# yynps737/zero-latency-yolo

Measured on AMD Instinct MI355X. Metric: frames_per_sec, higher is better.
Workload: dtype bf16; 1 GPU; YOLOv8-nano 416x416 batch=64 throughput path (BASELINE configs[2]), bf16; engines_per_gpu=3, weights=seeded synthetic (no real weights offline), graph=True, parallelism=single GPU

## Files before the change

### zero-latency-yolo_amd/csrc/engine.cpp

```cpp
#include "zly_internal.h"
#include "weights.h"

#include <algorithm>
#include <atomic>
#include <chrono>
#include <condition_variable>
#include <deque>
#include <map>
#include <mutex>
#include <string>
#include <thread>
#include <type_traits>
#include <vector>
#include <string.h>
#include <stdio.h>
#include <stdlib.h>

namespace zly {

static thread_local std::string g_last_error;

static int fail(int code, const std::string& msg) { g_last_error = msg; return code; }

#define HIP_TRY(expr, code)                                                                        \
// ... 2392 lines not shown
    HIP_TRY(hipMemcpyAsync(out, e->d_scratch_f32, elems * sizeof(float), hipMemcpyDeviceToHost, e->stream), ZLY_ERR_INFERENCE);
    HIP_TRY(hipStreamSynchronize(e->stream), ZLY_ERR_INFERENCE);
    if (c) *c = C;
    if (h) *h = b.H;
    if (w) *w = b.W;
    return ZLY_OK;
}

int32_t zly_num_classes(const zly_engine* e) { return e ? e->nc : 0; }
int32_t zly_weights_fp8(const zly_engine* e) { return (e && e->model.fp8_weights) ? 1 : 0; }
int32_t zly_num_anchors(const zly_engine* e) { return e ? e->N : 0; }
int32_t zly_num_ops(const zly_engine* e) { return e ? (int32_t)e->ops.size() : 0; }

int32_t zly_op_info_at(const zly_engine* e, int32_t i, zly_op_info* out)
{
    if (!e || !out || i < 0 || i >= (int32_t)e->ops.size()) return fail(ZLY_ERR_INVALID_ARGUMENT, "bad argument");
    const Op& op = e->ops[(size_t)i];
    memset(out, 0, sizeof *out);
    snprintf(out->name, sizeof out->name, "%s", op.name.c_str());
    out->kind = op.kind;
    out->flops_per_frame = op.flops;
    out->bytes_per_frame = op.bytes;
    return ZLY_OK;
}

int32_t zly_op_kernel_name(zly_engine* e, int32_t i, int32_t n, char* out, size_t cap)
{
    if (!e || !out || cap < 8 || i < 0 || i >= (int32_t)e->ops.size() || n < 1 || n > e->cfg.max_batch) return fail(ZLY_ERR_INVALID_ARGUMENT, "bad argument");
    std::lock_guard<std::mutex> lk(e->mu);
    const std::vector<Launch>& t = resolve_launches(e, n);
    const Launch& L = t[(size_t)i];
    const Op& op = e->ops[(size_t)i];
    std::string k;
    switch (L.kind) {
    case LK_NONE:
        switch (t[(size_t)L.covered_by].kind) {
        case LK_STEM: case LK_STEM1: k = op.kind == OP_PREPROCESS ? "(fused into stem_fused_kernel)" : "(fused into the previous launch)"; break;
        case LK_PAIR: case LK_WS_PAIR: k = "(fused into the previous launch)"; break;
        case LK_C2F: k = "(fused into the C2f kernel at " + e->ops[(size_t)L.covered_by].name + ")"; break;
        case LK_SPPF_FUSED: k = "(fused into the SPPF kernel at model.9.cv1)"; break;
        case LK_MULTI: k = "(in a merged Detect launch)"; break;
        case LK_HEAD: k = op.kind == OP_CONV ? "(computed in the Detect tail at surviving anchors)" : "(covered by the last tail launch)"; break;
        }
        break;
    case LK_PREPROCESS: k = L.lb ? "preprocess_kernel<LB> (letterbox)" : "preprocess_kernel"; break;
    case LK_STEM: k = L.lb ? "stem_fused_kernel<LB> (letterbox)" : "stem_fused_kernel"; break;
    case LK_STEM1: k = L.lb ? "stem_model1_kernel<LB> (letterbox preprocess+model.0+model.1)" : "stem_model1_kernel (preprocess+model.0+model.1)"; break;
    case LK_SPPF_POOL: k = L.pool16 ? "sppf_pool16_kernel<DPP row windows, one barrier>" : "sppf_pool_kernel"; break;
    case LK_SPPF_FUSED: k = "sppf_fused_kernel<cv1+3 pools+cv2,SPLIT=" + std::to_string(sppf_split(e->ops[(size_t)e->sppf_cv2].cout, n, e->sw)) + ">"; break;
    case LK_MULTI: k = L.multi_ct == 3 ? "conv_igemm_multi_kernel<CT=3> (the 3 Detect stems)" : "conv_igemm_multi_kernel<CT=2> (the 6 Detect branch convs)"; break;
    case LK_C2F: {
        const C2fGroup& g = e->c2fs[(size_t)op.c2f];
        k = "c2f_kernel<C=" + std::to_string(g.c) + (g.c == 32 ? ",NW=" + std::to_string(L.c2f.nw) : std::string()) +
            (g.mode == 3 ? ",cv1+bottleneck+cv2>" : g.mode == 1 ? ",cv1+bottleneck>" : ",bottleneck+cv2>");
        break;
    }
    case LK_PAIR: k = "bottleneck_pair_kernel<" + std::to_string(e->pairs[(size_t)op.pair].c) + ">"; break;
    case LK_WS_PAIR: k = std::string("conv3x3_ws_pair_kernel<") + (e->pairs[(size_t)op.pair].res ? "RES," : "") + "64->64->64," + std::to_string(L.ws_pair.g.TH) + "x" + std::to_string(L.ws_pair.g.TW) + " tiles>"; break;
    case LK_CONV_WSK: k = "conv3x3_wsk_kernel<K=720 packed across taps,5 channel tiles>"; break;
    case LK_CONV: {
        const int cin = op.in.C + (op.in2.buf >= 0 ? op.in2.C : 0);
        const ConvPlan& c = L.conv;
        switch (c.kind) {
        case CONV_WS1: k = std::string("conv1x1_ws_kernel<") + (op.in2.buf >= 0 ? "dual-source," : "") + "NK=" + std::to_string(cin / 32) + "," + std::to_string(c.ct) + " channel tiles," + std::to_string(c.pt * 16) + " px>"; break;
        case CONV_WS: k = std::string("conv3x3_ws_kernel<") + (op.stride == 2 ? "S=2," : "") + (c.rowt ? "ROWT," : "") + (c.tpw1 ? "TPW=1," : "TPW=2,") + std::to_string(c.ct) + " channel tiles>"; break;
        case CONV_LDS: k = "conv3x3_lds_kernel<S=" + std::to_string(op.stride) + ",CT=" + std::to_string(c.ct) + ",PT=" + std::to_string(c.pt) + (c.wres ? ",wres>" : ">"); break;
        case CONV_STREAM: k = "conv1x1_stream_kernel<CT=" + std::to_string(c.ct) + ",PT=" + std::to_string(c.pt) + ",NK=" + std::to_string((cin + 31) / 32) + ">"; break;
        default: k = std::string("conv_igemm_kernel<") + (op.ks == 1 ? (op.in2.buf >= 0 ? "1x1 dual-source" : "1x1") : (c.fastk ? "3x3" : "3x3 generic-K")) +
                 ",CT=" + std::to_string(c.ct) + ",PT=" + std::to_string(c.pt) + ",KSPLIT=" + std::to_string(c.ksplit) + ">";
        }
        break;
    }
    case LK_HEAD: {
        k = L.lb ? "head_fused_kernel<LB> (letterbox box mapping)" : "head_fused_kernel";
        std::string lv;
        for (int l = 0; l < 3; ++l)
            if (L.box_mode[l] && (L.only_level < 0 || L.only_level == l)) lv += std::string(lv.empty() ? "" : ",") + "P" + std::to_string(3 + l) + (L.box_mode[l] == 1 ? ":ws" : ":lds");
        if (!lv.empty()) k += " (+ box conv in k-step order " + lv + ")";
        break;
    }
    case LK_NMS: k = "nms_kernel"; break;
    }
    snprintf(out, cap, "%s", k.c_str());
    return ZLY_OK;
}

int32_t zly_launch_info_at(zly_engine* e, int32_t i, int32_t n, zly_launch_info* out)
{
    if (!e || !out || i < 0 || i >= (int32_t)e->ops.size() || n < 1 || n > e->cfg.max_batch) return fail(ZLY_ERR_INVALID_ARGUMENT, "bad argument");
    std::lock_guard<std::mutex> lk(e->mu);
    memset(out, 0, sizeof *out);
    const int nops = (int)e->ops.size();
    const std::vector<Launch>& t = resolve_launches(e, n);
    out->covered_by = t[(size_t)i].covered_by;
    if (out->covered_by != i) return ZLY_OK;
    std::vector<char> in_group((size_t)nops, 0);
    for (int j = 0; j < nops; ++j) in_group[(size_t)j] = t[(size_t)j].covered_by == i ? 1 : 0;
    std::map<int, std::vector<char>> written_in, read_out, counted_in, counted_out;
    auto chan = [&](std::map<int, std::vector<char>>& m, int buf) -> std::vector<char>& {
        std::vector<char>& v = m[buf];
        if (v.empty()) v.assign((size_t)e->bufs[(size_t)buf].C + 64, 0);
        return v;
    };
    std::vector<IoView> io;
    for (int j = 0; j < nops; ++j) {
        io.clear();
        if (in_group[(size_t)j]) { op_writes(e, e->ops[(size_t)j], &io); for (const IoView& v : io) for (int c = 0; c < v.C; ++c) chan(written_in, v.buf)[(size_t)(v.co + c)] = 1; }
// ... 108 lines not shown
```

### zero-latency-yolo_amd/csrc/kernels_pair.hip

```cpp
#include "zly_internal.h"
#include "conv_device.h"
#include <stdlib.h>
#include <stdio.h>

namespace zly {

typedef __attribute__((ext_vector_type(4))) short s16x4;
typedef __attribute__((ext_vector_type(4))) unsigned int u32x4_t;

template <int C> struct PairGeom;
template <> struct PairGeom<16> {
    static constexpr int CT = 1, KS = 1, FRAGB = 8, PITCH = 48, WTILE = 512;
    static constexpr bool WRES = true;
    typedef s16x4 frag;
    static __device__ __forceinline__ f32x4 mma(frag a, frag b, f32x4 c) { return __builtin_amdgcn_mfma_f32_16x16x16bf16_1k(a, b, c, 0, 0, 0); }
};
template <> struct PairGeom<32> {
    static constexpr int CT = 2, KS = 1, FRAGB = 16, PITCH = 96, WTILE = 1024;
    static constexpr bool WRES = true;
    typedef bf16x8 frag;
    static __device__ __forceinline__ f32x4 mma(frag a, frag b, f32x4 c) { return __builtin_amdgcn_mfma_f32_16x16x32_bf16(a, b, c, 0, 0, 0); }
};
template <> struct PairGeom<64> {
    static constexpr int CT = 4, KS = 2, FRAGB = 16, PITCH = 160, WTILE = 1024;
    static constexpr bool WRES = false;
    typedef bf16x8 frag;
    static __device__ __forceinline__ f32x4 mma(frag a, frag b, f32x4 c) { return __builtin_amdgcn_mfma_f32_16x16x32_bf16(a, b, c, 0, 0, 0); }
};

__device__ __forceinline__ int div_small(int q, float inv) { return (int)(((float)q + 0.5f) * inv); }

template <int C>
__device__ __forceinline__ void pair_taps(const unsigned char* __restrict__ src, const unsigned char* __restrict__ lw, int off, int rowb, int lane,
                                          f32x4 (&acc)[PairGeom<C>::CT])
{
    typedef PairGeom<C> G;
    typedef typename G::frag F;
#pragma unroll
    for (int c = 0; c < G::CT; ++c) acc[c] = f32x4{0.f, 0.f, 0.f, 0.f};
    const unsigned char* wl = lw + lane * G::FRAGB;
    const int kxo[3] = {0, G::FRAGB == 8 ? opaque_offset(G::PITCH) : G::PITCH, G::FRAGB == 8 ? opaque_offset(2 * G::PITCH) : 2 * G::PITCH};
#pragma unroll
    for (int ky = 0; ky < 3; ++ky) {
        const unsigned char* row = src + off + ky * rowb;
#pragma unroll
        for (int kx = 0; kx < 3; ++kx) {
#pragma unroll
            for (int ks = 0; ks < G::KS; ++ks) {
                const F x = *reinterpret_cast<const F*>(row + (G::FRAGB == 8 ? kxo[kx] : kx * G::PITCH) + ks * 64);
#pragma unroll
                for (int c = 0; c < G::CT; ++c) {
                    const F w = *reinterpret_cast<const F*>(wl + ((c * 9 + ky * 3 + kx) * G::KS + ks) * G::WTILE);
                    acc[c] = G::mma(w, x, acc[c]);
                }
            }
        }
// ... 121 lines not shown
            stage_weights(lwB, a.wB);
            __syncthreads();
        }

        for (int t = wave; t < ntB; t += NW) {
            if (C == 64) asm volatile("" ::: "memory");
            const int q = t * 16 + p;
            const int qc = min(q, NPB - 1);
            const int oy = div_small(qc, invTW), ox = qc - oy * a.TW;
            f32x4 acc[G::CT];
            pair_taps<C>(lmid, lwB, (oy * MW + ox) * G::PITCH + kq * G::FRAGB, MW * G::PITCH, lane, acc);
            f32x4 o[G::CT];
#pragma unroll
            for (int c = 0; c < G::CT; ++c) {
                f32x4 v = acc[c] + biasB[c];
#pragma unroll
                for (int r = 0; r < 4; ++r) v[r] = silu<bf16_t>(v[r]);
                o[c] = v;
            }
            const int gy = y0 + oy, gx = x0 + ox;
            if (q < NPB && gy < a.H && gx < a.W) {
                const unsigned char* xs = lin + ((oy + 2) * PW + ox + 2) * G::PITCH;
                bf16_t* dst = out + ((size_t)(b * a.H + gy) * a.W + gx) * a.out_cs;
                if (C == 16) {
                    if (a.res) o[0] += load4(reinterpret_cast<const bf16_t*>(xs) + kq * 4);
                    store4(dst + kq * 4, o[0]);
                } else {
#pragma unroll
                    for (int g2 = 0; g2 < G::CT / 2; ++g2) {
                        f32x4 lo = o[2 * g2], hi = o[(2 * g2 + 1) % G::CT];
                        if (a.res) {
                            f32x4 ra, rb;
                            load8(reinterpret_cast<const bf16_t*>(xs) + g2 * 32 + kq * 8, ra, rb);
                            lo += ra; hi += rb;
                        }
                        store8(dst + g2 * 32 + kq * 8, lo, hi);
                    }
                }
            }
        }
        if (tnext >= a.total_tiles) break;
        tl = tnext;
        __syncthreads();
    }
}

#ifdef ZLY_C2F_DIAG
__device__ unsigned long long* g_c2f_diag = nullptr;
#define C2FSTAMP(k) do { __builtin_amdgcn_sched_barrier(0); unsigned long long t_; asm volatile("s_memtime %0\n\ts_waitcnt lgkmcnt(0)" : "=s"(t_) :: "memory"); dsum[k] += t_ - dT0; dT0 = t_; __builtin_amdgcn_sched_barrier(0); } while (0)
#else
#define C2FSTAMP(k) do { } while (0)
#endif
static constexpr int C2F_BIAS_BYTES = 1024;
template <int C, int MODE, int NW, int NLD, int NK1>
__global__ __launch_bounds__(NW * 64) void c2f_kernel(const C2fArgs a)
{
    typedef PairGeom<C> G;
    typedef typename G::frag F;
    constexpr bool FRONT = (MODE & 1) != 0, BACK = (MODE & 2) != 0;
    constexpr int NT = NW * 64;
    constexpr int UPP = C / 8;
    constexpr int WBYTES = 9 * G::CT * G::WTILE;
    constexpr int T1 = 2 * C / 16;
    constexpr int T2MAX = 4;
    extern __shared__ __attribute__((aligned(16))) unsigned char smem[];
#ifdef ZLY_C2F_DIAG
    unsigned long long dsum[12] = {0, 0, 0, 0, 0, 0, 0, 0, 0, 0, 0, 0}, dT0 = __builtin_amdgcn_s_memtime();
    const unsigned long long dstart = dT0;
#endif
    const int PW = a.TW + 4, PH = a.TH + 4, MW = a.TW + 2, MH = a.TH + 2;
    const int w1_bytes = FRONT ? T1 * a.nk1 * 1024 : 0;
    const int T2 = a.Cout2 >> 4;
    const int w2_bytes = BACK ? T2 * a.nk2 * G::WTILE : 0;
    float* lbias = reinterpret_cast<float*>(smem);
    unsigned char* lwA = smem + C2F_BIAS_BYTES;
    unsigned char* lwB = lwA + WBYTES;
    unsigned char* lw1 = lwB + WBYTES;
    unsigned char* lw2 = lw1 + w1_bytes;
    unsigned char* lin = lw2 + w2_bytes;
    unsigned char* lmid = lin + (PH * PW * G::PITCH + 15) / 16 * 16;
    unsigned char* ly2 = lmid + (MH * MW * G::PITCH + 15) / 16 * 16;
    unsigned char* ly0 = ly2 + (BACK ? (a.TH * a.TW * G::PITCH + 15) / 16 * 16 : 0);

    const int tid = threadIdx.x, lane = tid & 63;
    const int wave = __builtin_amdgcn_readfirstlane(tid >> 6);
    const int p = lane & 15, kq = lane >> 4;
    bf16_t* __restrict__ cat = static_cast<bf16_t*>(a.cat);

    auto stage = [&](unsigned char* dst, const void* src, int bytes) {
        for (int u = tid; u < bytes / 16; u += NT)
            *reinterpret_cast<u32x4_t*>(dst + (size_t)u * 16) = *reinterpret_cast<const u32x4_t*>(static_cast<const unsigned char*>(src) + (size_t)u * 16);
    };
    stage(lwA, a.wA, WBYTES);
    stage(lwB, a.wB, WBYTES);
    if (FRONT) stage(lw1, a.w1, w1_bytes);
    if (BACK) stage(lw2, a.w2, w2_bytes);

    constexpr bool BIAS_LDS = C == 32 && NW == 16;
    if (BIAS_LDS) {
        for (int u = tid; u < C; u += NT) { lbias[u] = a.bA[u]; lbias[C + u] = a.bB[u]; }
        if (FRONT) for (int u = tid; u < 2 * C; u += NT) lbias[2 * C + u] = a.b1[u];
        if (BACK) for (int u = tid; u < a.Cout2; u += NT) lbias[4 * C + u] = a.b2[u];
    }
    constexpr int NBR = BIAS_LDS ? 1 : G::CT, NB1 = BIAS_LDS ? 1 : T1, NB2 = BIAS_LDS ? 1 : T2MAX;
    f32x4 rbA[NBR], rbB[NBR], rb1[NB1], rb2[NB2];
    if (!BIAS_LDS) {
#pragma unroll
        for (int c = 0; c < G::CT; ++c) {
            const int ch = C == 16 ? kq * 4 : (c >> 1) * 32 + kq * 8 + (c & 1) * 4;
            rbA[c % NBR] = *reinterpret_cast<const f32x4*>(a.bA + ch);
            rbB[c % NBR] = *reinterpret_cast<const f32x4*>(a.bB + ch);
        }
#pragma unroll
        for (int c = 0; c < T1; ++c) {
            const int ch = C == 16 ? c * 16 + kq * 4 : (c >> 1) * 32 + kq * 8 + (c & 1) * 4;
            rb1[c % NB1] = FRONT ? *reinterpret_cast<const f32x4*>(a.b1 + ch) : f32x4{0.f, 0.f, 0.f, 0.f};
        }
#pragma unroll
        for (int c = 0; c < T2MAX; ++c)
            rb2[c % NB2] = (BACK && c < T2) ? *reinterpret_cast<const f32x4*>(a.b2 + (c >> 1) * 32 + kq * 8 + (c & 1) * 4) : f32x4{0.f, 0.f, 0.f, 0.f};
    }
    auto bias_of = [&](int which, int c) -> f32x4 {
        if (BIAS_LDS) {
            const int base = which == 0 ? 0 : which == 1 ? C : which == 2 ? 2 * C : 4 * C;
            return *reinterpret_cast<const f32x4*>(lbias + base + (c >> 1) * 32 + kq * 8 + (c & 1) * 4);
        }
        return which == 0 ? rbA[c % NBR] : which == 1 ? rbB[c % NBR] : which == 2 ? rb1[c % NB1] : rb2[c % NB2];
    };
    const float invPW = 1.0f / (float)PW, invMW = 1.0f / (float)MW, invTW = 1.0f / (float)a.TW;
    const int tiles_per_img = a.tiles_x * a.tiles_y;
    const int NP0 = PH * PW, NPA = MH * MW, NPB = a.TH * a.TW;
    const int nt0 = (NP0 + 15) >> 4, ntA = (NPA + 15) >> 4, ntB = (NPB + 15) >> 4;
    const int NPU = NP0 * UPP;

    auto tile_origin = [&](int tl, int& b, int& y0, int& x0) {
        b = tl / tiles_per_img;
        const int r = tl - b * tiles_per_img;
        const int ty = r / a.tiles_x;
        y0 = ty * a.TH; x0 = (r - ty * a.tiles_x) * a.TW;
    };
    auto put_map = [&](unsigned char* dst, const f32x4* o) {
        if (C == 16) store4(reinterpret_cast<bf16_t*>(dst) + kq * 4, o[0]);
        else store8(reinterpret_cast<bf16_t*>(dst) + kq * 8, o[0], o[1]);
    };
    const __amdgpu_buffer_rsrc_t rcat = __builtin_amdgcn_make_buffer_rsrc(a.cat, 0, (unsigned)((size_t)a.n * a.H * a.W * a.cat_cs * 2), 0x00020000);
    auto put_global = [&](int elem, const f32x4* o) {
        if (C == 16) {
            const bf16x4 v = to_bf16x4(o[0]);
            typedef __attribute__((ext_vector_type(2))) unsigned int u32x2_t;
            __builtin_amdgcn_raw_buffer_store_b64(__builtin_bit_cast(u32x2_t, v), rcat, (elem + kq * 4) * 2, 0, 0);
        } else {
            const bf16x8 v = to_bf16x8(o[0], o[1]);
            __builtin_amdgcn_raw_buffer_store_b128(__builtin_bit_cast(u32x4_t, v), rcat, (elem + kq * 8) * 2, 0, 0);
        }
    };

    u32x4_t pre[NLD];
    auto stage_load = [&](int tl) {
        int b, y0, x0;
        tile_origin(tl, b, y0, x0);
        const bf16_t* in = cat + a.pair_in_co;
#pragma unroll
        for (int i = 0; i < NLD; ++i) {
            const int u = tid + i * NT;
            u32x4_t v = {0u, 0u, 0u, 0u};
            if (u < NPU) {
                const int px = u / UPP, part = u - px * UPP;
                const int py = div_small(px, invPW), pxx = px - py * PW;
                const int gy = y0 - 2 + py, gx = x0 - 2 + pxx;
                if ((unsigned)gy < (unsigned)a.H && (unsigned)gx < (unsigned)a.W)
                    v = *reinterpret_cast<const u32x4_t*>(in + ((size_t)(b * a.H + gy) * a.W + gx) * a.cat_cs + part * 8);
            }
            pre[i] = v;
        }
    };
    auto stage_store = [&]() {
#pragma unroll
        for (int i = 0; i < NLD; ++i) {
            const int u = tid + i * NT;
            if (u < NPU) {
                const int px = u / UPP, part = u - px * UPP;
                *reinterpret_cast<u32x4_t*>(lin + px * G::PITCH + part * 16) = pre[i];
            }
        }
    };

    int tl = blockIdx.x;
    if (tl >= a.total_tiles) return;
    if (!FRONT) stage_load(tl);
    C2FSTAMP(0);
    while (true) {
        int b, y0, x0;
        tile_origin(tl, b, y0, x0);
        const int tnext = tl + gridDim.x;
        if (!FRONT) {
            stage_store();
            __syncthreads();
            C2FSTAMP(1);
            if (tnext < a.total_tiles) stage_load(tnext);
        } else {
            const bf16_t* __restrict__ xa = static_cast<const bf16_t*>(a.x) + a.x_co;
            const bf16_t* __restrict__ xb = static_cast<const bf16_t*>(a.x2) + a.x2_co;
            const bool dual = a.x2 != nullptr;
            const unsigned char* w1l = lw1 + lane * 16;
            auto load_x = [&](int t, bf16x8 (&xf)[NK1]) {
                const int qc = min(t * 16 + p, NP0 - 1);
                const int py = div_small(qc, invPW), px = qc - py * PW;
                const int gy = y0 - 2 + py, gx = x0 - 2 + px;
                const bool inimg = (unsigned)gy < (unsigned)a.H && (unsigned)gx < (unsigned)a.W;
                const size_t pa = dual ? ((size_t)(b * (a.H >> 1) + (gy >> 1)) * (a.W >> 1) + (gx >> 1)) * a.x_cs : ((size_t)(b * a.H + gy) * a.W + gx) * a.x_cs;
                const size_t pb2 = ((size_t)(b * a.H + gy) * a.W + gx) * a.x2_cs;
#pragma unroll
                for (int s = 0; s < NK1; ++s) {
                    const int ci = s * 32 + kq * 8;
#pragma unroll
                    for (int j = 0; j < 8; ++j) xf[s][j] = (bf16_t)0.0f;
                    if (inimg) xf[s] = (dual && ci >= a.split_c) ? *reinterpret_cast<const bf16x8*>(xb + pb2 + (ci - a.split_c)) : *reinterpret_cast<const bf16x8*>(xa + pa + ci);
                }
            };
            bf16x8 xcur[NK1], xnext[NK1];
            if (wave < nt0) load_x(wave, xcur);
            __syncthreads();
            C2FSTAMP(1);
            for (int t = wave; t < nt0; t += NW) {
                if (t + NW < nt0) load_x(t + NW, xnext);
                const int q = t * 16 + p;
                const int qc = min(q, NP0 - 1);
                const int py = div_small(qc, invPW), px = qc - py * PW;
                const int gy = y0 - 2 + py, gx = x0 - 2 + px;
                const bool inimg = (unsigned)gy < (unsigned)a.H && (unsigned)gx < (unsigned)a.W;
                f32x4 acc[T1];
#pragma unroll
                for (int c = 0; c < T1; ++c) acc[c] = f32x4{0.f, 0.f, 0.f, 0.f};
#pragma unroll
                for (int s = 0; s < NK1; ++s)
#pragma unroll
                    for (int c = 0; c < T1; ++c) {
                        const bf16x8 wf = *reinterpret_cast<const bf16x8*>(w1l + (c * NK1 + s) * 1024);
                        acc[c] = __builtin_amdgcn_mfma_f32_16x16x32_bf16(wf, xcur[s], acc[c], 0, 0, 0);
                    }
#pragma unroll
                for (int s = 0; s < NK1; ++s) xcur[s] = xnext[s];
                f32x4 o[T1];
#pragma unroll
                for (int c = 0; c < T1; ++c) {
                    f32x4 v = acc[c] + bias_of(2, c);
#pragma unroll
                    for (int r = 0; r < 4; ++r) v[r] = inimg ? silu<bf16_t>(v[r]) : 0.0f;
                    o[c] = v;
                }
                if (q < NP0) {
                    put_map(lin + (size_t)qc * G::PITCH, o + G::CT);
                    const int iy = py - 2, ix = px - 2;
                    const bool interior = (unsigned)iy < (unsigned)a.TH && (unsigned)ix < (unsigned)a.TW && inimg;
                    if (interior) {
                        if (MODE == 3) put_map(ly0 + (size_t)(iy * a.TW + ix) * G::PITCH, o);
                        if (MODE == 1 || a.dump) {
                            const int dst = ((b * a.H + gy) * a.W + gx) * a.cat_cs;
                            put_global(dst, o);
                            put_global(dst + C, o + G::CT);
                        }
                    }
                }
            }
            C2FSTAMP(2);
            __syncthreads();
            C2FSTAMP(3);
        }

        for (int t = wave; t < ntA; t += NW) {
            const int q = t * 16 + p;
            const int qc = min(q, NPA - 1);
            const int my = div_small(qc, invMW), mx = qc - my * MW;
            f32x4 acc[G::CT];
            pair_taps<C>(lin, lwA, (my * PW + mx) * G::PITCH + kq * G::FRAGB, PW * G::PITCH, lane, acc);
            const int gy = y0 - 1 + my, gx = x0 - 1 + mx;
            const bool inimg = (unsigned)gy < (unsigned)a.H && (unsigned)gx < (unsigned)a.W;
            f32x4 o[G::CT];
#pragma unroll
            for (int c = 0; c < G::CT; ++c) {
                f32x4 v = acc[c] + bias_of(0, c);
#pragma unroll
                for (int r = 0; r < 4; ++r) v[r] = inimg ? silu<bf16_t>(v[r]) : 0.0f;
                o[c] = v;
            }
            if (q < NPA) put_map(lmid + (size_t)(my * MW + mx) * G::PITCH, o);
        }
        C2FSTAMP(4);
        __syncthreads();
        C2FSTAMP(5);

        for (int t = wave; t < ntB; t += NW) {
            const int q = t * 16 + p;
            const int qc = min(q, NPB - 1);
            const int oy = div_small(qc, invTW), ox = qc - oy * a.TW;
            f32x4 acc[G::CT];
            pair_taps<C>(lmid, lwB, (oy * MW + ox) * G::PITCH + kq * G::FRAGB, MW * G::PITCH, lane, acc);
            f32x4 o[G::CT];
#pragma unroll
            for (int c = 0; c < G::CT; ++c) {
                f32x4 v = acc[c] + bias_of(1, c);
#pragma unroll
                for (int r = 0; r < 4; ++r) v[r] = silu<bf16_t>(v[r]);
                o[c] = v;
            }
            const int gy = y0 + oy, gx = x0 + ox;
            if (q < NPB) {
                if (a.res) {
                    const unsigned char* xs = lin + ((oy + 2) * PW + ox + 2) * G::PITCH;
                    if (C == 16) o[0] += load4(reinterpret_cast<const bf16_t*>(xs) + kq * 4);
                    else { f32x4 ra, rb; load8(reinterpret_cast<const bf16_t*>(xs) + kq * 8, ra, rb); o[0] += ra; o[1 % G::CT] += rb; }
                }
                if (BACK) put_map(ly2 + (size_t)qc * G::PITCH, o);
                if ((!BACK || a.dump) && gy < a.H && gx < a.W)
                    put_global(((b * a.H + gy) * a.W + gx) * a.cat_cs + a.pair_out_co, o);
            }
        }

        C2FSTAMP(6);
        if (BACK) {
            __syncthreads();
            C2FSTAMP(7);
            const unsigned char* w2l = lw2 + lane * G::FRAGB;
            for (int t = wave; t < ntB; t += NW) {
                const int q = t * 16 + p;
                const int qc = min(q, NPB - 1);
                const int oy = div_small(qc, invTW), ox = qc - oy * a.TW;
                const int gy = min(y0 + oy, a.H - 1), gx = min(x0 + ox, a.W - 1);
                const bf16_t* gp = cat + ((size_t)(b * a.H + gy) * a.W + gx) * a.cat_cs + kq * (G::FRAGB / 2);
                constexpr int NS = MODE == 2 ? 4 : 3;
                F xs[NS];
                if (MODE == 2) {
                    xs[0] = *reinterpret_cast<const F*>(gp);
                    xs[1] = *reinterpret_cast<const F*>(gp + C);
                } else {
                    xs[0] = *reinterpret_cast<const F*>(ly0 + (size_t)qc * G::PITCH + kq * G::FRAGB);
                }
                xs[NS - 2] = *reinterpret_cast<const F*>(lin + (size_t)((oy + 2) * PW + ox + 2) * G::PITCH + kq * G::FRAGB);
                xs[NS - 1] = *reinterpret_cast<const F*>(ly2 + (size_t)qc * G::PITCH + kq * G::FRAGB);
                f32x4 acc[T2MAX];
#pragma unroll
                for (int c = 0; c < T2MAX; ++c) acc[c] = f32x4{0.f, 0.f, 0.f, 0.f};
#pragma unroll
                for (int s = 0; s < NS; ++s)
#pragma unroll
                    for (int c = 0; c < T2MAX; ++c)
                        if (c < T2) acc[c] = G::mma(*reinterpret_cast<const F*>(w2l + (c * NS + s) * G::WTILE), xs[s], acc[c]);
                if (q < NPB && y0 + oy < a.H && x0 + ox < a.W) {
                    bf16_t* dst = static_cast<bf16_t*>(a.out) + ((size_t)(b * a.H + gy) * a.W + gx) * a.out_cs + a.out_co;
#pragma unroll
                    for (int g2 = 0; g2 < T2MAX / 2; ++g2) {
                        if (2 * g2 >= T2) break;
                        f32x4 lo = acc[2 * g2] + bias_of(3, 2 * g2), hi = acc[2 * g2 + 1] + bias_of(3, 2 * g2 + 1);
#pragma unroll
                        for (int r = 0; r < 4; ++r) { lo[r] = silu<bf16_t>(lo[r]); hi[r] = silu<bf16_t>(hi[r]); }
                        store8(dst + g2 * 32 + kq * 8, lo, hi);
                    }
                }
            }
        }
        C2FSTAMP(8);
        if (tnext >= a.total_tiles) break;
        tl = tnext;
        if (!FRONT) __syncthreads();
    }
#ifdef ZLY_C2F_DIAG
    if (lane == 0 && g_c2f_diag) {
        unsigned long long* o = g_c2f_diag + ((size_t)blockIdx.x * NW + wave) * 16;
        for (int i = 0; i < 9; ++i) o[i] = dsum[i];
        o[9] = __builtin_amdgcn_s_memtime() - dstart;
    }
#endif
}

static constexpr int PAIR_NW16 = 16, PAIR_NW32 = 8, PAIR_NW64 = 8, PAIR_NLD = 4, PAIR_NLD64 = 6;
static int pair_nw(int c) { return c == 16 ? PAIR_NW16 : PAIR_NW32; }
static int pair_nld(int c) { return c == 64 ? PAIR_NLD64 : PAIR_NLD; }
static constexpr int PAIR_LDS_MAX = 160 * 1024;

static int pair_pitch(int c) { return c == 16 ? PairGeom<16>::PITCH : c == 32 ? PairGeom<32>::PITCH : PairGeom<64>::PITCH; }
static int pair_wbytes_total(int c) { return c == 16 ? 2 * 9 * PairGeom<16>::WTILE : c == 32 ? 2 * 9 * 2 * PairGeom<32>::WTILE : 9 * 2 * 4 * PairGeom<64>::WTILE; }
static size_t pair_lds_bytes(int c, int th, int tw)
{
    const size_t pitch = (size_t)pair_pitch(c);
    return (size_t)pair_wbytes_total(c) + ((size_t)(th + 4) * (tw + 4) * pitch + 15) / 16 * 16 + (size_t)(th + 2) * (tw + 2) * pitch;
}

bool pair_plan(int c, int n, int H, int W, const Switches& sw, PairPlan* plan)
{
    if (c != 16 && c != 32 && c != 64) return false;
    const int ncu = sw.num_cus, nw = pair_nw(c);
    double best = 1e30;
    for (int th = 4; th <= 32; ++th) {
        for (int tw = 8; tw <= 64; ++tw) {
            if (pair_lds_bytes(c, th, tw) > (size_t)PAIR_LDS_MAX) continue;
            if ((th + 4) * (tw + 4) * (c / 8) > nw * 64 * pair_nld(c)) continue;
            const int tx = (W + tw - 1) / tw, ty = (H + th - 1) / th;
            const long tiles = (long)n * tx * ty;
            const long rounds = (tiles + ncu - 1) / ncu;
            const int ntA = ((th + 2) * (tw + 2) + 15) / 16, ntB = (th * tw + 15) / 16;
            const double per_tile = (double)((ntA + nw - 1) / nw + (ntB + nw - 1) / nw) + 1.5 * 16 / nw;
            const double cost = (double)rounds * per_tile;
            if (cost < best) { best = cost; plan->th = th; plan->tw = tw; plan->tiles_x = tx; plan->tiles_y = ty; plan->total_tiles = (int)tiles; }
        }
    }
    if (best >= 1e30) return false;
    plan->grid = plan->total_tiles < ncu ? plan->total_tiles : ncu;
    plan->lds_bytes = (int)pair_lds_bytes(c, plan->th, plan->tw);
    return true;
}

hipError_t pair_init()
{
    hipError_t r = hipFuncSetAttribute((const void*)bottleneck_pair_kernel<16, PAIR_NW16, PAIR_NLD>, hipFuncAttributeMaxDynamicSharedMemorySize, PAIR_LDS_MAX);
    if (r != hipSuccess) return r;
    r = hipFuncSetAttribute((const void*)bottleneck_pair_kernel<32, PAIR_NW32, PAIR_NLD>, hipFuncAttributeMaxDynamicSharedMemorySize, PAIR_LDS_MAX);
    if (r != hipSuccess) return r;
    return hipFuncSetAttribute((const void*)bottleneck_pair_kernel<64, PAIR_NW64, PAIR_NLD64>, hipFuncAttributeMaxDynamicSharedMemorySize, PAIR_LDS_MAX);
}

static constexpr int C2F_NW16 = 16, C2F_NW32 = 8, C2F_NLD = 4;
static int c2f_nw32(int mode, const Switches& sw)
{
    if (sw.c2f32_nw == 8 || sw.c2f32_nw == 16) return sw.c2f32_nw;
    return mode == 1 ? C2F_NW32 : 16;
}
static size_t c2f_lds_bytes(int c, int mode, int nk1, int nk2, int cout2, int th, int tw)
{
    const size_t pitch = (size_t)pair_pitch(c), wtile = c == 16 ? 512 : 1024, ct = c / 16;
    size_t b = C2F_BIAS_BYTES + 2 * 9 * ct * wtile;
    if (mode & 1) b += (size_t)(2 * c / 16) * nk1 * 1024;
    if (mode & 2) b += (size_t)(cout2 / 16) * nk2 * wtile;
    b += ((size_t)(th + 4) * (tw + 4) * pitch + 15) / 16 * 16 + ((size_t)(th + 2) * (tw + 2) * pitch + 15) / 16 * 16;
    if (mode & 2) b += ((size_t)th * tw * pitch + 15) / 16 * 16;
    if (mode == 3) b += ((size_t)th * tw * pitch + 15) / 16 * 16;
    return b;
}

typedef void (*c2f_fn)(const C2fArgs);
static c2f_fn pick_c2f(int c, int mode, int nk1, int nw32);

bool c2f_plan(int c, int mode, int nk1, int nk2, int cout2, int n, int H, int W, const Switches& sw, C2fPlan* plan)
{
    if (c == 64 && mode >= 1 && mode <= 3) return c2f64_plan(mode, nk1, nk2, cout2, n, H, W, sw, plan);
    if ((c != 16 && c != 32) || mode < 1 || mode > 3 || !pick_c2f(c, mode, nk1, c2f_nw32(mode, sw))) return false;
    if ((mode & 2) && nk2 != (mode == 2 ? 4 : 3)) return false;
    const int ncu = sw.num_cus, nw = c == 16 ? C2F_NW16 : c2f_nw32(mode, sw);
    const size_t lds_cap = sw.c2f_lds_kb ? (size_t)sw.c2f_lds_kb * 1024 : (size_t)PAIR_LDS_MAX;
    double best = 1e30;
    for (int th = 4; th <= 32; ++th) {
        for (int tw = 8; tw <= 64; ++tw) {
            if (c2f_lds_bytes(c, mode, nk1, nk2, cout2, th, tw) > lds_cap) continue;
            if (sw.c2f_tile_th && (sw.c2f_tile_th != th || sw.c2f_tile_tw != tw)) continue;
            if (!(mode & 1) && (th + 4) * (tw + 4) * (c / 8) > nw * 64 * C2F_NLD) continue;
            const int tx = (W + tw - 1) / tw, ty = (H + th - 1) / th;
            const long tiles = (long)n * tx * ty;
            const long rounds = (tiles + ncu - 1) / ncu;
            const int nt0 = ((th + 4) * (tw + 4) + 15) / 16, ntA = ((th + 2) * (tw + 2) + 15) / 16, ntB = (th * tw + 15) / 16;
            const int ct = c / 16;
            const double w_cv1 = (double)(2 * ct * nk1 + 2.0 * 2 * ct) / (9.0 * ct + 2.0 * ct);
            const double w_cv2 = (double)((cout2 / 16) * nk2 + 2.0 * (cout2 / 16)) / (9.0 * ct + 2.0 * ct);
            double per_tile = (double)((ntA + nw - 1) / nw + (ntB + nw - 1) / nw) + 1.5 * 16 / nw;
            if (mode & 1) per_tile += w_cv1 * ((nt0 + nw - 1) / nw);
            if (mode & 2) per_tile += w_cv2 * ((ntB + nw - 1) / nw);
            const double cost = (double)rounds * per_tile;
            if (cost < best) { best = cost; plan->th = th; plan->tw = tw; plan->tiles_x = tx; plan->tiles_y = ty; plan->total_tiles = (int)tiles; }
        }
    }
    if (best >= 1e30) return false;
    plan->grid = plan->total_tiles < ncu ? plan->total_tiles : ncu;
    plan->lds_bytes = (int)c2f_lds_bytes(c, mode, nk1, nk2, cout2, plan->th, plan->tw);
    plan->nw = nw;
    return true;
}

template <int C, int NW> static c2f_fn pick_c2f_c(int mode, int nk1)
{
    if (mode == 2) return c2f_kernel<C, 2, NW, C2F_NLD, 1>;
    if (mode == 1) return nk1 == 1 ? c2f_kernel<C, 1, NW, C2F_NLD, 1> : nk1 == 2 ? c2f_kernel<C, 1, NW, C2F_NLD, 2> : nk1 == 6 ? c2f_kernel<C, 1, NW, C2F_NLD, 6> : nullptr;
    return nk1 == 1 ? c2f_kernel<C, 3, NW, C2F_NLD, 1> : nk1 == 2 ? c2f_kernel<C, 3, NW, C2F_NLD, 2> : nk1 == 6 ? c2f_kernel<C, 3, NW, C2F_NLD, 6> : nullptr;
}
static c2f_fn pick_c2f(int c, int mode, int nk1, int nw32)
{
    return c == 16 ? pick_c2f_c<16, C2F_NW16>(mode, nk1) : nw32 == 16 ? pick_c2f_c<32, 16>(mode, nk1) : pick_c2f_c<32, C2F_NW32>(mode, nk1);
}

hipError_t c2f_init()
{
    static const int nk1s[3] = {1, 2, 6};
    for (int c = 16; c <= 32; c += 16)
        for (int mode = 1; mode <= 3; ++mode)
            for (int i = 0; i < 3; ++i)
                for (int nw32 = 8; nw32 <= 16; nw32 += 8) {
                    hipError_t r = hipFuncSetAttribute((const void*)pick_c2f(c, mode, nk1s[i], nw32), hipFuncAttributeMaxDynamicSharedMemorySize, PAIR_LDS_MAX);
                    if (r != hipSuccess) return r;
                }
    return c2f64_init();
}

hipError_t launch_c2f(int c, int mode, const C2fArgs& a, const C2fPlan& plan, hipStream_t s)
{
    if (c == 64) return launch_c2f64(mode, a, plan, s);
    if ((c != 16 && c != 32) || mode < 1 || mode > 3 || a.TH != plan.th || a.TW != plan.tw || plan.grid < 1) return hipErrorInvalidValue;
    if (a.cat_cs % 8 || a.pair_in_co % c || a.pair_out_co % c || a.out_cs % 8 || a.out_co % 8) return hipErrorInvalidValue;
    if ((mode & 1) && (a.x_cs % 8 || a.x_co % 8 || (a.x2 && (a.x2_cs % 8 || a.x2_co % 8 || a.split_c % 32 || (a.H & 1) || (a.W & 1))))) return hipErrorInvalidValue;
    if ((mode & 2) && (a.Cout2 % 32 || a.Cout2 > 64)) return hipErrorInvalidValue;
    const int nw = c == 16 ? C2F_NW16 : plan.nw;
    if (c == 32 && nw != 8 && nw != 16) return hipErrorInvalidValue;
    c2f_fn fn = pick_c2f(c, mode, a.nk1, nw);
    if (!fn || (mode == 2 && a.pair_in_co != 2 * c)) return hipErrorInvalidValue;
    hipLaunchKernelGGL(fn, dim3((unsigned)plan.grid), dim3(nw * 64), (size_t)plan.lds_bytes, s, a);
    return hipGetLastError();
}

hipError_t launch_pair(int c, const PairArgs& a, const PairPlan& plan, hipStream_t s)
{
    if ((c != 16 && c != 32 && c != 64) || a.TH != plan.th || a.TW != plan.tw || plan.grid < 1) return hipErrorInvalidValue;
    if (a.in_cs % 8 || a.in_co % 8 || a.out_cs % 8 || a.out_co % 8) return hipErrorInvalidValue;
    if (c == 16) hipLaunchKernelGGL((bottleneck_pair_kernel<16, PAIR_NW16, PAIR_NLD>), dim3((unsigned)plan.grid), dim3(PAIR_NW16 * 64), (size_t)plan.lds_bytes, s, a);
    else if (c == 32) hipLaunchKernelGGL((bottleneck_pair_kernel<32, PAIR_NW32, PAIR_NLD>), dim3((unsigned)plan.grid), dim3(PAIR_NW32 * 64), (size_t)plan.lds_bytes, s, a);
    else         hipLaunchKernelGGL((bottleneck_pair_kernel<64, PAIR_NW64, PAIR_NLD64>), dim3((unsigned)plan.grid), dim3(PAIR_NW64 * 64), (size_t)plan.lds_bytes, s, a);
    return hipGetLastError();
}

}
```

Before: 114,600 frames/s.

## Keep C2f y2 in registers, skip redundant ring cv1 work, prefetch cv2 inputs

For C=32 C2f kernels, the bottleneck output y2 now stays in registers instead of going through an LDS buffer. This removes a barrier and the LDS round-trip and frees LDS for larger tiles. In mode 3 the cv1 stage splits into a halo-ring pass and an interior pass, so the ring only computes the channels the bottleneck needs. cv2 inputs are prefetched one tile ahead, and the tile planner's cost model is updated to match. The changes add register pressure and code complexity, and they cap tile size at four carried tiles per wave.

```diff
diff --git a/zero-latency-yolo_amd/csrc/engine.cpp b/zero-latency-yolo_amd/csrc/engine.cpp
--- a/zero-latency-yolo_amd/csrc/engine.cpp
+++ b/zero-latency-yolo_amd/csrc/engine.cpp
@@ -2468,7 +2468,7 @@
     case LK_C2F: {
         const C2fGroup& g = e->c2fs[(size_t)op.c2f];
         k = "c2f_kernel<C=" + std::to_string(g.c) + (g.c == 32 ? ",NW=" + std::to_string(L.c2f.nw) : std::string()) +
-            (g.mode == 3 ? ",cv1+bottleneck+cv2>" : g.mode == 1 ? ",cv1+bottleneck>" : ",bottleneck+cv2>");
+            (g.mode == 3 ? ",cv1+bottleneck+cv2," : g.mode == 1 ? ",cv1+bottleneck," : ",bottleneck+cv2,") + std::to_string(L.c2f.th) + "x" + std::to_string(L.c2f.tw) + " tiles>";
         break;
     }
     case LK_PAIR: k = "bottleneck_pair_kernel<" + std::to_string(e->pairs[(size_t)op.pair].c) + ">"; break;
diff --git a/zero-latency-yolo_amd/csrc/kernels_pair.hip b/zero-latency-yolo_amd/csrc/kernels_pair.hip
--- a/zero-latency-yolo_amd/csrc/kernels_pair.hip
+++ b/zero-latency-yolo_amd/csrc/kernels_pair.hip
@@ -2,6 +2,7 @@
 #include "conv_device.h"
 #include <stdlib.h>
 #include <stdio.h>
+#include <type_traits>
 
 namespace zly {
 
@@ -229,12 +230,17 @@
 #define C2FSTAMP(k) do { } while (0)
 #endif
 static constexpr int C2F_BIAS_BYTES = 1024;
+static constexpr bool c2f_ring(int c, int mode) { return c == 32 && mode == 3; }
+static constexpr bool c2f_y2reg(int c, int mode) { return c == 32 && (mode & 2) != 0; }
+static constexpr bool c2f_tight(int c, int nw) { return c == 32 && nw == 16; }
+static constexpr int C2F_MAXY = 4;
 template <int C, int MODE, int NW, int NLD, int NK1>
 __global__ __launch_bounds__(NW * 64) void c2f_kernel(const C2fArgs a)
 {
     typedef PairGeom<C> G;
     typedef typename G::frag F;
     constexpr bool FRONT = (MODE & 1) != 0, BACK = (MODE & 2) != 0;
+    constexpr bool RING = c2f_ring(C, MODE), Y2REG = c2f_y2reg(C, MODE), TIGHT = c2f_tight(C, NW);
     constexpr int NT = NW * 64;
     constexpr int UPP = C / 8;
     constexpr int WBYTES = 9 * G::CT * G::WTILE;
@@ -257,7 +263,7 @@
     unsigned char* lin = lw2 + w2_bytes;
     unsigned char* lmid = lin + (PH * PW * G::PITCH + 15) / 16 * 16;
     unsigned char* ly2 = lmid + (MH * MW * G::PITCH + 15) / 16 * 16;
-    unsigned char* ly0 = ly2 + (BACK ? (a.TH * a.TW * G::PITCH + 15) / 16 * 16 : 0);
+    unsigned char* ly0 = ly2 + (BACK && !Y2REG ? (a.TH * a.TW * G::PITCH + 15) / 16 * 16 : 0);
 
     const int tid = threadIdx.x, lane = tid & 63;
     const int wave = __builtin_amdgcn_readfirstlane(tid >> 6);
@@ -307,7 +313,10 @@
     const float invPW = 1.0f / (float)PW, invMW = 1.0f / (float)MW, invTW = 1.0f / (float)a.TW;
     const int tiles_per_img = a.tiles_x * a.tiles_y;
     const int NP0 = PH * PW, NPA = MH * MW, NPB = a.TH * a.TW;
-    const int nt0 = (NP0 + 15) >> 4, ntA = (NPA + 15) >> 4, ntB = (NPB + 15) >> 4;
+    const int ntA = (NPA + 15) >> 4, ntB = (NPB + 15) >> 4;
+    const int NPR = RING ? 4 * PW + 4 * a.TH : 0;
+    const int NPI = RING ? NPB : NP0;
+    const int ntR = (NPR + 15) >> 4, nt0 = ntR + ((NPI + 15) >> 4);
     const int NPU = NP0 * UPP;
 
     auto tile_origin = [&](int tl, int& b, int& y0, int& x0) {
@@ -376,20 +385,42 @@
             C2FSTAMP(1);
             if (tnext < a.total_tiles) stage_load(tnext);
         } else {
+            const int pF = TIGHT ? opaque_offset(p) : p, kqF = TIGHT ? opaque_offset(kq) : kq, laneF = TIGHT ? opaque_offset(lane) : lane;
             const bf16_t* __restrict__ xa = static_cast<const bf16_t*>(a.x) + a.x_co;
             const bf16_t* __restrict__ xb = static_cast<const bf16_t*>(a.x2) + a.x2_co;
             const bool dual = a.x2 != nullptr;
-            const unsigned char* w1l = lw1 + lane * 16;
+            const unsigned char* w1l = lw1 + laneF * 16;
+            auto cv1_pixel = [&](int t, int& py, int& px) -> bool {
+                if (RING && t < ntR) {
+                    const int q = t * 16 + pF, r = min(q, NPR - 1);
+                    if (r < 4 * PW) {
+                        const int row = div_small(r, invPW);
+                        px = r - row * PW; py = row < 2 ? row : row + a.TH;
+                    } else {
+                        const int s = r - 4 * PW, col = s & 3;
+                        py = 2 + (s >> 2); px = col < 2 ? col : col + a.TW;
+                    }
+                    return q < NPR;
+                }
+                const int q = (t - ntR) * 16 + pF, j = min(q, NPI - 1);
+                if (RING) {
+                    const int iy = div_small(j, invTW);
+                    py = iy + 2; px = j - iy * a.TW + 2;
+                } else {
+                    py = div_small(j, invPW); px = j - py * PW;
+                }
+                return q < NPI;
+            };
             auto load_x = [&](int t, bf16x8 (&xf)[NK1]) {
-                const int qc = min(t * 16 + p, NP0 - 1);
-                const int py = div_small(qc, invPW), px = qc - py * PW;
+                int py, px;
+                cv1_pixel(t, py, px);
                 const int gy = y0 - 2 + py, gx = x0 - 2 + px;
                 const bool inimg = (unsigned)gy < (unsigned)a.H && (unsigned)gx < (unsigned)a.W;
                 const size_t pa = dual ? ((size_t)(b * (a.H >> 1) + (gy >> 1)) * (a.W >> 1) + (gx >> 1)) * a.x_cs : ((size_t)(b * a.H + gy) * a.W + gx) * a.x_cs;
                 const size_t pb2 = ((size_t)(b * a.H + gy) * a.W + gx) * a.x2_cs;
 #pragma unroll
                 for (int s = 0; s < NK1; ++s) {
-                    const int ci = s * 32 + kq * 8;
+                    const int ci = s * 32 + kqF * 8;
 #pragma unroll
                     for (int j = 0; j < 8; ++j) xf[s][j] = (bf16_t)0.0f;
                     if (inimg) xf[s] = (dual && ci >= a.split_c) ? *reinterpret_cast<const bf16x8*>(xb + pb2 + (ci - a.split_c)) : *reinterpret_cast<const bf16x8*>(xa + pa + ci);
@@ -399,39 +430,36 @@
             if (wave < nt0) load_x(wave, xcur);
             __syncthreads();
             C2FSTAMP(1);
-            for (int t = wave; t < nt0; t += NW) {
-                if (t + NW < nt0) load_x(t + NW, xnext);
-                const int q = t * 16 + p;
-                const int qc = min(q, NP0 - 1);
-                const int py = div_small(qc, invPW), px = qc - py * PW;
-                const int gy = y0 - 2 + py, gx = x0 - 2 + px;
-                const bool inimg = (unsigned)gy < (unsigned)a.H && (unsigned)gx < (unsigned)a.W;
+            auto cv1_tile = [&](auto c0, int t) {
+                constexpr int C0 = decltype(c0)::value;
                 f32x4 acc[T1];
 #pragma unroll
-                for (int c = 0; c < T1; ++c) acc[c] = f32x4{0.f, 0.f, 0.f, 0.f};
+                for (int c = C0; c < T1; ++c) acc[c] = f32x4{0.f, 0.f, 0.f, 0.f};
 #pragma unroll
                 for (int s = 0; s < NK1; ++s)
 #pragma unroll
-                    for (int c = 0; c < T1; ++c) {
+                    for (int c = C0; c < T1; ++c) {
                         const bf16x8 wf = *reinterpret_cast<const bf16x8*>(w1l + (c * NK1 + s) * 1024);
                         acc[c] = __builtin_amdgcn_mfma_f32_16x16x32_bf16(wf, xcur[s], acc[c], 0, 0, 0);
                     }
 #pragma unroll
                 for (int s = 0; s < NK1; ++s) xcur[s] = xnext[s];
+                int py, px;
+                const bool valid = cv1_pixel(t, py, px);
+                const int gy = y0 - 2 + py, gx = x0 - 2 + px;
+                const bool inimg = (unsigned)gy < (unsigned)a.H && (unsigned)gx < (unsigned)a.W;
                 f32x4 o[T1];
 #pragma unroll
-                for (int c = 0; c < T1; ++c) {
+                for (int c = C0; c < T1; ++c) {
                     f32x4 v = acc[c] + bias_of(2, c);
 #pragma unroll
                     for (int r = 0; r < 4; ++r) v[r] = inimg ? silu<bf16_t>(v[r]) : 0.0f;
                     o[c] = v;
                 }
-                if (q < NP0) {
-                    put_map(lin + (size_t)qc * G::PITCH, o + G::CT);
-                    const int iy = py - 2, ix = px - 2;
-                    const bool interior = (unsigned)iy < (unsigned)a.TH && (unsigned)ix < (unsigned)a.TW && inimg;
-                    if (interior) {
-                        if (MODE == 3) put_map(ly0 + (size_t)(iy * a.TW + ix) * G::PITCH, o);
+                if (valid) {
+                    put_map(lin + (size_t)(py * PW + px) * G::PITCH, o + G::CT);
+                    if (C0 == 0 && inimg && (RING || ((unsigned)(py - 2) < (unsigned)a.TH && (unsigned)(px - 2) < (unsigned)a.TW))) {
+                        if (MODE == 3) put_map(ly0 + (size_t)((py - 2) * a.TW + px - 2) * G::PITCH, o);
                         if (MODE == 1 || a.dump) {
                             const int dst = ((b * a.H + gy) * a.W + gx) * a.cat_cs;
                             put_global(dst, o);
@@ -439,18 +467,24 @@
                         }
                     }
                 }
+            };
+            for (int t = wave; t < nt0; t += NW) {
+                if (t + NW < nt0) load_x(t + NW, xnext);
+                if (RING && t < ntR) cv1_tile(std::integral_constant<int, G::CT>(), t);
+                else cv1_tile(std::integral_constant<int, 0>(), t);
             }
             C2FSTAMP(2);
             __syncthreads();
             C2FSTAMP(3);
         }
 
+        const int pA = TIGHT ? opaque_offset(p) : p, kqA = TIGHT ? opaque_offset(kq) : kq, laneA = TIGHT ? opaque_offset(lane) : lane;
         for (int t = wave; t < ntA; t += NW) {
-            const int q = t * 16 + p;
+            const int q = t * 16 + pA;
             const int qc = min(q, NPA - 1);
             const int my = div_small(qc, invMW), mx = qc - my * MW;
             f32x4 acc[G::CT];
-            pair_taps<C>(lin, lwA, (my * PW + mx) * G::PITCH + kq * G::FRAGB, PW * G::PITCH, lane, acc);
+            pair_taps<C>(lin, lwA, (my * PW + mx) * G::PITCH + kqA * G::FRAGB, PW * G::PITCH, laneA, acc);
             const int gy = y0 - 1 + my, gx = x0 - 1 + mx;
             const bool inimg = (unsigned)gy < (unsigned)a.H && (unsigned)gx < (unsigned)a.W;
             f32x4 o[G::CT];
@@ -467,12 +501,40 @@
         __syncthreads();
         C2FSTAMP(5);
 
-        for (int t = wave; t < ntB; t += NW) {
-            const int q = t * 16 + p;
+        constexpr int NS = MODE == 2 ? 4 : 3;
+        const int pB = TIGHT ? opaque_offset(p) : p, kqB = TIGHT ? opaque_offset(kq) : kq, laneB = TIGHT ? opaque_offset(lane) : lane;
+        constexpr int NY = Y2REG ? C2F_MAXY : 1;
+        F y2f[NY], xs2[NS - 1], xs2n[NS - 1];
+#pragma unroll
+        for (int i = 0; i < NY; ++i) y2f[i] = F{};
+#pragma unroll
+        for (int s = 0; s < NS - 1; ++s) xs2n[s] = F{};
+        auto y2_put = [&](int i, F v) {
+            static_assert(C2F_MAXY == 4, "one branch per carried tile");
+            if (i == 0) y2f[0] = v; else if (i == 1) y2f[1 % NY] = v; else if (i == 2) y2f[2 % NY] = v; else y2f[3 % NY] = v;
+        };
+        auto y2_get = [&](int i) -> F { return i == 0 ? y2f[0] : i == 1 ? y2f[1 % NY] : i == 2 ? y2f[2 % NY] : y2f[3 % NY]; };
+        auto load_cv2 = [&](int t, F (&x)[NS - 1]) {
+            const int qc = min(t * 16 + pB, NPB - 1);
+            const int oy = div_small(qc, invTW), ox = qc - oy * a.TW;
+            if (MODE == 2) {
+                const int gy = min(y0 + oy, a.H - 1), gx = min(x0 + ox, a.W - 1);
+                const bf16_t* gp = cat + ((size_t)(b * a.H + gy) * a.W + gx) * a.cat_cs + kqB * (G::FRAGB / 2);
+                x[0] = *reinterpret_cast<const F*>(gp);
+                x[1] = *reinterpret_cast<const F*>(gp + C);
+            } else {
+                x[0] = *reinterpret_cast<const F*>(ly0 + (size_t)qc * G::PITCH + kqB * G::FRAGB);
+            }
+            x[NS - 2] = *reinterpret_cast<const F*>(lin + (size_t)((oy + 2) * PW + ox + 2) * G::PITCH + kqB * G::FRAGB);
+        };
+        if (Y2REG) load_cv2(wave, xs2);
+        auto conv_b_tile = [&](int t, int i) {
+            if (BACK && TIGHT) asm volatile("" ::: "memory");
+            const int q = t * 16 + pB;
             const int qc = min(q, NPB - 1);
             const int oy = div_small(qc, invTW), ox = qc - oy * a.TW;
             f32x4 acc[G::CT];
-            pair_taps<C>(lmid, lwB, (oy * MW + ox) * G::PITCH + kq * G::FRAGB, MW * G::PITCH, lane, acc);
+            pair_taps<C>(lmid, lwB, (oy * MW + ox) * G::PITCH + kqB * G::FRAGB, MW * G::PITCH, laneB, acc);
             f32x4 o[G::CT];
 #pragma unroll
             for (int c = 0; c < G::CT; ++c) {
@@ -482,39 +544,33 @@
                 o[c] = v;
             }
             const int gy = y0 + oy, gx = x0 + ox;
-            if (q < NPB) {
-                if (a.res) {
-                    const unsigned char* xs = lin + ((oy + 2) * PW + ox + 2) * G::PITCH;
-                    if (C == 16) o[0] += load4(reinterpret_cast<const bf16_t*>(xs) + kq * 4);
-                    else { f32x4 ra, rb; load8(reinterpret_cast<const bf16_t*>(xs) + kq * 8, ra, rb); o[0] += ra; o[1 % G::CT] += rb; }
-                }
-                if (BACK) put_map(ly2 + (size_t)qc * G::PITCH, o);
-                if ((!BACK || a.dump) && gy < a.H && gx < a.W)
-                    put_global(((b * a.H + gy) * a.W + gx) * a.cat_cs + a.pair_out_co, o);
-            }
-        }
+            if (a.res) {
+                const unsigned char* xs = lin + ((oy + 2) * PW + ox + 2) * G::PITCH;
+                if (C == 16) o[0] += load4(reinterpret_cast<const bf16_t*>(xs) + kqB * 4);
+                else { f32x4 ra, rb; load8(reinterpret_cast<const bf16_t*>(xs) + kqB * 8, ra, rb); o[0] += ra; o[1 % G::CT] += rb; }
+            }
+            if constexpr (Y2REG) {
+                if constexpr (C == 16) y2_put(i, __builtin_bit_cast(F, to_bf16x4(o[0])));
+                else y2_put(i, __builtin_bit_cast(F, to_bf16x8(o[0], o[1 % G::CT])));
+            } else if (BACK && q < NPB) put_map(ly2 + (size_t)qc * G::PITCH, o);
+            if ((!BACK || a.dump) && q < NPB && gy < a.H && gx < a.W)
+                put_global(((b * a.H + gy) * a.W + gx) * a.cat_cs + a.pair_out_co, o);
+        };
+        for (int t = wave, i = 0; t < ntB; t += NW, ++i) conv_b_tile(t, i);
 
         C2FSTAMP(6);
         if (BACK) {
-            __syncthreads();
+            if (!Y2REG) __syncthreads();
             C2FSTAMP(7);
-            const unsigned char* w2l = lw2 + lane * G::FRAGB;
-            for (int t = wave; t < ntB; t += NW) {
-                const int q = t * 16 + p;
+            const unsigned char* w2l = lw2 + laneB * G::FRAGB;
+            for (int t = wave, i = 0; t < ntB; t += NW, ++i) {
+                if (!Y2REG) load_cv2(t, xs2);
+                else if (t + NW < ntB) load_cv2(t + NW, xs2n);
+                const int q = t * 16 + pB;
                 const int qc = min(q, NPB - 1);
+                const F yf = Y2REG ? y2_get(i) : *reinterpret_cast<const F*>(ly2 + (size_t)qc * G::PITCH + kqB * G::FRAGB);
                 const int oy = div_small(qc, invTW), ox = qc - oy * a.TW;
                 const int gy = min(y0 + oy, a.H - 1), gx = min(x0 + ox, a.W - 1);
-                const bf16_t* gp = cat + ((size_t)(b * a.H + gy) * a.W + gx) * a.cat_cs + kq * (G::FRAGB / 2);
-                constexpr int NS = MODE == 2 ? 4 : 3;
-                F xs[NS];
-                if (MODE == 2) {
-                    xs[0] = *reinterpret_cast<const F*>(gp);
-                    xs[1] = *reinterpret_cast<const F*>(gp + C);
-                } else {
-                    xs[0] = *reinterpret_cast<const F*>(ly0 + (size_t)qc * G::PITCH + kq * G::FRAGB);
-                }
-                xs[NS - 2] = *reinterpret_cast<const F*>(lin + (size_t)((oy + 2) * PW + ox + 2) * G::PITCH + kq * G::FRAGB);
-                xs[NS - 1] = *reinterpret_cast<const F*>(ly2 + (size_t)qc * G::PITCH + kq * G::FRAGB);
                 f32x4 acc[T2MAX];
 #pragma unroll
                 for (int c = 0; c < T2MAX; ++c) acc[c] = f32x4{0.f, 0.f, 0.f, 0.f};
@@ -522,7 +578,11 @@
                 for (int s = 0; s < NS; ++s)
 #pragma unroll
                     for (int c = 0; c < T2MAX; ++c)
-                        if (c < T2) acc[c] = G::mma(*reinterpret_cast<const F*>(w2l + (c * NS + s) * G::WTILE), xs[s], acc[c]);
+                        if (c < T2) acc[c] = G::mma(*reinterpret_cast<const F*>(w2l + (c * NS + s) * G::WTILE), s < NS - 1 ? xs2[s < NS - 1 ? s : 0] : yf, acc[c]);
+                if (Y2REG) {
+#pragma unroll
+                    for (int s = 0; s < NS - 1; ++s) xs2[s] = xs2n[s];
+                }
                 if (q < NPB && y0 + oy < a.H && x0 + ox < a.W) {
                     bf16_t* dst = static_cast<bf16_t*>(a.out) + ((size_t)(b * a.H + gy) * a.W + gx) * a.out_cs + a.out_co;
 #pragma unroll
@@ -531,7 +591,7 @@
                         f32x4 lo = acc[2 * g2] + bias_of(3, 2 * g2), hi = acc[2 * g2 + 1] + bias_of(3, 2 * g2 + 1);
 #pragma unroll
                         for (int r = 0; r < 4; ++r) { lo[r] = silu<bf16_t>(lo[r]); hi[r] = silu<bf16_t>(hi[r]); }
-                        store8(dst + g2 * 32 + kq * 8, lo, hi);
+                        store8(dst + g2 * 32 + kqB * 8, lo, hi);
                     }
                 }
             }
@@ -609,7 +669,7 @@
     if (mode & 1) b += (size_t)(2 * c / 16) * nk1 * 1024;
     if (mode & 2) b += (size_t)(cout2 / 16) * nk2 * wtile;
     b += ((size_t)(th + 4) * (tw + 4) * pitch + 15) / 16 * 16 + ((size_t)(th + 2) * (tw + 2) * pitch + 15) / 16 * 16;
-    if (mode & 2) b += ((size_t)th * tw * pitch + 15) / 16 * 16;
+    if ((mode & 2) && !c2f_y2reg(c, mode)) b += ((size_t)th * tw * pitch + 15) / 16 * 16;
     if (mode == 3) b += ((size_t)th * tw * pitch + 15) / 16 * 16;
     return b;
 }
@@ -630,16 +690,22 @@
             if (c2f_lds_bytes(c, mode, nk1, nk2, cout2, th, tw) > lds_cap) continue;
             if (sw.c2f_tile_th && (sw.c2f_tile_th != th || sw.c2f_tile_tw != tw)) continue;
             if (!(mode & 1) && (th + 4) * (tw + 4) * (c / 8) > nw * 64 * C2F_NLD) continue;
+            if (c2f_y2reg(c, mode) && (th * tw + 15) / 16 > nw * C2F_MAXY) continue;
             const int tx = (W + tw - 1) / tw, ty = (H + th - 1) / th;
             const long tiles = (long)n * tx * ty;
             const long rounds = (tiles + ncu - 1) / ncu;
-            const int nt0 = ((th + 4) * (tw + 4) + 15) / 16, ntA = ((th + 2) * (tw + 2) + 15) / 16, ntB = (th * tw + 15) / 16;
+            const bool ring = c2f_ring(c, mode);
+            const int ntR = ring ? (4 * (tw + 4) + 4 * th + 15) / 16 : 0, nt1 = ((ring ? th * tw : (th + 4) * (tw + 4)) + 15) / 16, ntA = ((th + 2) * (tw + 2) + 15) / 16, ntB = (th * tw + 15) / 16;
             const int ct = c / 16;
             const double w_cv1 = (double)(2 * ct * nk1 + 2.0 * 2 * ct) / (9.0 * ct + 2.0 * ct);
             const double w_cv2 = (double)((cout2 / 16) * nk2 + 2.0 * (cout2 / 16)) / (9.0 * ct + 2.0 * ct);
             double per_tile = (double)((ntA + nw - 1) / nw + (ntB + nw - 1) / nw) + 1.5 * 16 / nw;
-            if (mode & 1) per_tile += w_cv1 * ((nt0 + nw - 1) / nw);
+            if (mode & 1) {
+                const int ring0 = (ntR + nw - 1) / nw, all0 = (ntR + nt1 + nw - 1) / nw;
+                per_tile += w_cv1 * (0.5 * ring0 + (all0 - ring0));
+            }
             if (mode & 2) per_tile += w_cv2 * ((ntB + nw - 1) / nw);
+            if (c2f_y2reg(c, mode) && tiles > ncu) per_tile += 1e-5 * (th + 4) * (tw + 4);
             const double cost = (double)rounds * per_tile;
             if (cost < best) { best = cost; plan->th = th; plan->tw = tw; plan->tiles_x = tx; plan->tiles_y = ty; plan->total_tiles = (int)tiles; }
         }
@@ -684,6 +750,7 @@
     if ((mode & 2) && (a.Cout2 % 32 || a.Cout2 > 64)) return hipErrorInvalidValue;
     const int nw = c == 16 ? C2F_NW16 : plan.nw;
     if (c == 32 && nw != 8 && nw != 16) return hipErrorInvalidValue;
+    if (c2f_y2reg(c, mode) && (a.TH * a.TW + 15) / 16 > nw * C2F_MAXY) return hipErrorInvalidValue;
     c2f_fn fn = pick_c2f(c, mode, a.nk1, nw);
     if (!fn || (mode == 2 && a.pair_in_co != 2 * c)) return hipErrorInvalidValue;
     hipLaunchKernelGGL(fn, dim3((unsigned)plan.grid), dim3(nw * 64), (size_t)plan.lds_bytes, s, a);
```

Measured after the change: 115,900 frames/s, median of 6. 1.01x the previous value.
